# XingqunQi-lab/EmotionGestures

Hardware: AMD Instinct MI355X
Metric: gesture clips/sec (34 frames, 43 joints) (higher is better)
Workload: dtype bf16x3; 1 GPU; TED clips: 4 s 16 kHz audio -> mel(128x124) -> CVAE sample -> generator -> 34x126 pose; global_batch=64, variant=Models_spatial_memory, parallelism=clip-sharded x1, no data-path collective, launch=hipGraph replay, 4 step(s) in flight, branch_streams=False, fold_affine=False

## Files before the change

### emotiongestures_amd/csrc/conv.hip

```cpp
#include <type_traits>
#include "common.h"


namespace {

struct ConvArgs {
    const float* x; const float* w; const float* bias; const float* scale; const float* shift;
    float* y; float* gap;
    float* gap2 = nullptr;
    int H, W, Ho, Wo, cout, relu, nchw, tiles_x, tiles;
    const float* gate = nullptr; const float* res = nullptr; int relu2 = 0;
    const float* in_scale = nullptr; const float* in_shift = nullptr;
    int wrow = 0;
    const unsigned* res_bits = nullptr;
    const float* res_q = nullptr;
    unsigned int* dbg = nullptr;
    const float* sc_x = nullptr; const bf8* sc_whi = nullptr; const bf8* sc_wlo = nullptr; const float* sc_vec = nullptr;
    int sc_H = 0, sc_W = 0, sc_S = 2, sc_B = 0;
};
__device__ __forceinline__ f4 residual_quad(const float* __restrict__ res, const unsigned* __restrict__ bits, size_t e) {
    f4 r = *reinterpret_cast<const f4*>(res + e);
    if (bits) {
        const unsigned nb = bits[e >> 5] >> (unsigned)(e & 28);
        r[0] = (nb & 1u) ? r[0] : 0.f;
        r[1] = (nb & 2u) ? r[1] : 0.f;
        r[2] = (nb & 4u) ? r[2] : 0.f;
        r[3] = (nb & 8u) ? r[3] : 0.f;
    }
    return r;
}

template <int S, int TH> struct ConvGeom {
    static constexpr int IH = (TH - 1) * S + 3;
    static constexpr int IW = 31 * S + 3;
    static constexpr int NPIX = IH * IW;
    static constexpr int PL = (S == 1) ? ((NPIX + 15) / 16 * 16) : (NPIX | 1);
    static constexpr int MT = TH * 2 / 4;
};

template <int TH> struct ConvGeomDG2 {
    static constexpr int IH = TH + 1;
    static constexpr int IW = 33;
    static constexpr int NPIX = IH * IW;
    static constexpr int PL = (NPIX + 15) / 16 * 16;
};

template <int CIN, int NT, int S, int TH>
__global__ __launch_bounds__(256) void conv3x3_f32_kernel(ConvArgs a) {
    using G = ConvGeom<S, TH>;
    constexpr int COUTP = NT * 16, IW = G::IW, NPIX = G::NPIX, PL = G::PL, MT = G::MT;
    __shared__ f4 tile[8 * PL];

    const int tid = threadIdx.x, wave = tid >> 6, lane = tid & 63, li = lane & 15, kq = lane >> 4;
    int tile_id = blockIdx.x, b = blockIdx.y;
    {
        const int total = gridDim.x * gridDim.y;
        if ((total & 7) == 0) {
            const int lin = blockIdx.y * gridDim.x + blockIdx.x;
            const int log = (lin & 7) * (total >> 3) + (lin >> 3);
            b = log / (int)gridDim.x;
            tile_id = log - b * (int)gridDim.x;
        }
    }
    const int ty = tile_id / a.tiles_x, tx = tile_id - ty * a.tiles_x;
    const int oy0 = ty * TH, ox0 = tx * 32;
    const int iy0 = oy0 * S - 1, ix0 = ox0 * S - 1;

    int pbase[MT];
#pragma unroll
    for (int t = 0; t < MT; ++t) {
        const int id = wave * MT + t;
        pbase[t] = ((id >> 1) * S) * IW + ((id & 1) * 16 + li) * S;
    }
    f4 acc[MT][NT];
#pragma unroll
    for (int t = 0; t < MT; ++t)
#pragma unroll
        for (int n = 0; n < NT; ++n) acc[t][n] = (f4){0.f, 0.f, 0.f, 0.f};

    const f4* __restrict__ w4 = reinterpret_cast<const f4*>(a.w);
    const float* __restrict__ xb = a.x + (size_t)b * a.H * a.W * CIN;

    for (int chunk = 0; chunk < CIN / 32; ++chunk) {
        if (chunk) __syncthreads();
        for (int idx = tid; idx < ((NPIX + 7) / 8) * 64; idx += 256) {
            const int p = (idx >> 6) * 8 + (idx & 7), cq = (idx >> 3) & 7;
            if (p < NPIX) {
                const int iy = p / IW, ix = p - iy * IW;
                const int gy = iy0 + iy, gx = ix0 + ix;
                f4 v = (f4){0.f, 0.f, 0.f, 0.f};
                if (gy >= 0 && gy < a.H && gx >= 0 && gx < a.W)
                    v = *reinterpret_cast<const f4*>(xb + ((size_t)gy * a.W + gx) * CIN + chunk * 32 + cq * 4);
                tile[cq * PL + p] = v;
            }
        }
        __syncthreads();
        const f4* wp = w4 + (size_t)(chunk * 8 + kq) * COUTP + li;
#pragma unroll 1
        for (int kh = 0; kh < 3; ++kh) {
// ... 127 lines not shown
#pragma unroll
        for (int t = 0; t < MT; ++t)
#pragma unroll
            for (int n = 0; n < NT; ++n) acc[ph][t][n] = (f4){0.f, 0.f, 0.f, 0.f};
    const float* xb = a.x + (size_t)b * a.H * a.W * CIN;

    const int wave_u = __builtin_amdgcn_readfirstlane(wave);
    constexpr int PIECES = WIMG / 64;
    constexpr int GTOT = NIMG * PIECES;
    constexpr bool COUNTED = (GTOT % 4 == 0);
    constexpr int GW = GTOT / 4;
    auto issue_rows = [&](const bf8* __restrict__ ihi, const bf8* __restrict__ ilo, int row0, int buf) {
        if constexpr (SPLIT) {
            static_assert(COUNTED, "split instantiations deal whole pieces to the four waves");
            const size_t rbase = (size_t)row0 * a.wrow + c0;
#pragma unroll
            for (int p = 0; p < GW; ++p) {
                const int flat = p * 4 + wave_u;
                const int img = flat / PIECES, piece = flat - img * PIECES;
                const int slot = piece * 64 + lane, oct = slot / COUTP, co = slot - oct * COUTP;
                const bf8* src = (img ? ilo : ihi) + rbase + (size_t)oct * a.wrow + co;
                __builtin_amdgcn_global_load_lds((const __attribute__((address_space(1))) void*)src,
                                                 (__attribute__((address_space(3))) void*)(wring + buf * WBUF + img * WIMG + piece * 64), 16, 0, 0);
            }
            return;
        }
        const size_t gbase = (size_t)row0 * COUTP;
        if constexpr (PIECES % 4 == 0) {
#pragma unroll
            for (int img = 0; img < NIMG; ++img) {
                const bf8* src = (img ? ilo : ihi) + gbase;
#pragma unroll
                for (int p = 0; p < PIECES / 4; ++p) {
                    const int piece = p * 4 + wave_u;
                    __builtin_amdgcn_global_load_lds((const __attribute__((address_space(1))) void*)(src + piece * 64 + lane),
                                                     (__attribute__((address_space(3))) void*)(wring + buf * WBUF + img * WIMG + piece * 64),
                                                     16, 0, 0);
                }
            }
        } else {
#pragma unroll
            for (int p = 0; p < (GTOT + 3) / 4; ++p) {
                const int flat = p * 4 + wave_u;
                if (COUNTED || flat < GTOT) {
                    const int img = flat / PIECES, piece = flat - img * PIECES;
                    const bf8* src = (img ? ilo : ihi) + gbase;
                    __builtin_amdgcn_global_load_lds((const __attribute__((address_space(1))) void*)(src + piece * 64 + lane),
                                                     (__attribute__((address_space(3))) void*)(wring + buf * WBUF + img * WIMG + piece * 64),
                                                     16, 0, 0);
                }
            }
        }
    };
    auto issue_weights = [&](int step, int buf) {
        const int chunk = step / 9, tap = step - chunk * 9;
        issue_rows(whi, wlo, tap * (CIN / 8) + chunk * 4, buf);
    };
    constexpr int NIT = (((NPIX + 7) / 8) * 32 + 255) / 256;
    f4 pv[NIT][2];
    int goff[NIT], lslot[NIT];
    auto set_goff = [&](int toy0, int tox0) {
        const int iy0 = DG2 ? toy0 : toy0 * S - 1, ix0 = DG2 ? tox0 : tox0 * S - 1;
#pragma unroll
        for (int it = 0; it < NIT; ++it) {
            const int idx = tid + it * 256;
            const int p = (idx >> 5) * 8 + (idx & 7), oc = (idx >> 3) & 3;
            const int iy = p / IW, ix = p - iy * IW;
            const int gy = iy0 + iy, gx = ix0 + ix;
            const bool inside = p < NPIX && gy >= 0 && gy < a.H && gx >= 0 && gx < a.W;
            goff[it] = inside ? (gy * a.W + gx) * CIN + oc * 8 : -1;
            lslot[it] = p < NPIX ? oc * PL + p : -1;
        }
    };
    set_goff(oy0, ox0);
    auto load_tile = [&](int chunk) {
#pragma unroll
        for (int it = 0; it < NIT; ++it) {
            pv[it][0] = pv[it][1] = (f4){0.f, 0.f, 0.f, 0.f};
            if (goff[it] >= 0) {
                const float* src = xb + goff[it] + chunk * 32;
                pv[it][0] = *reinterpret_cast<const f4*>(src);
                pv[it][1] = *reinterpret_cast<const f4*>(src + 4);
            }
        }
    };
    const int oc8s = ((tid >> 3) & 3) * 8;
    auto store_tile = [&](int chunk) {
        f4 s0 = (f4){1.f, 1.f, 1.f, 1.f}, s1 = s0, h0 = (f4){0.f, 0.f, 0.f, 0.f}, h1 = h0;
        const bool in_aff = a.in_scale != nullptr;
        if (in_aff) {
            s0 = *reinterpret_cast<const f4*>(a.in_scale + chunk * 32 + oc8s); s1 = *reinterpret_cast<const f4*>(a.in_scale + chunk * 32 + oc8s + 4);
            h0 = *reinterpret_cast<const f4*>(a.in_shift + chunk * 32 + oc8s); h1 = *reinterpret_cast<const f4*>(a.in_shift + chunk * 32 + oc8s + 4);
        }
#pragma unroll
        for (int it = 0; it < NIT; ++it) {
            if (lslot[it] >= 0) {
                if (in_aff && goff[it] >= 0) {
                    pv[it][0] = pv[it][0] * s0 + h0;
                    pv[it][1] = pv[it][1] * s1 + h1;
                }
                bf8 hi, lo;
                split_octet<TERMS == 3>(pv[it][0], pv[it][1], hi, lo);
                tile[lslot[it]] = hi;
                if (TERMS == 3) tile[4 * PL + lslot[it]] = lo;
            }
        }
    };

// ... 64 lines not shown
            for (int it = 0; it < SNIT; ++it) {
                sv[it][0] = sv[it][1] = (f4){0.f, 0.f, 0.f, 0.f};
                if (sgoff[it] >= 0) {
                    const float* src = sxb + sgoff[it] + c * 32;
                    sv[it][0] = *reinterpret_cast<const f4*>(src);
                    sv[it][1] = *reinterpret_cast<const f4*>(src + 4);
                }
            }
        };
        load_sc(0);
        load_tile(0);
#pragma unroll
        for (int c = 0; c < SCC; ++c) {
#pragma unroll
            for (int it = 0; it < SNIT; ++it) {
                bf8 hi, lo;
                split_octet<TERMS == 3>(sv[it][0], sv[it][1], hi, lo);
                tile[sslot[it]] = hi;
                if (TERMS == 3) tile[4 * PL + sslot[it]] = lo;
            }
            if (c + 1 < SCC) load_sc(c + 1);
            __syncthreads();
            read_w(fr[0], 2 - c);
            read_x(fr[0], 4);
            mfma_half(fr[0], 0, 4);
            mfma_half(fr[0], 1, 4);
            __syncthreads();
        }
        if (SCC == 2) issue_weights(1, 1);
        const float* __restrict__ fv = a.sc_vec + (size_t)b * a.cout;
#pragma unroll
        for (int n = 0; n < NT; ++n) {
            const f4 fq = *reinterpret_cast<const f4*>(fv + c0 + (wn * NT + n) * 16 + kq * 4);
#pragma unroll
            for (int t = 0; t < MT; ++t) acc[0][t][n] = acc[0][t][n] * fq;
        }
    } else {
        issue_weights(0, 0);
        if (NSTEP > 1) issue_weights(1, 1);
        load_tile(0);
    }
#pragma unroll 1
    for (int chunk = 0; chunk < CIN / 32; ++chunk) {
        store_tile(chunk);
        if (COUNTED && chunk > 0) {
            wait_vmcnt_imm<GW>();
            wait_lgkmcnt0();
            wg_barrier();
        } else {
            __syncthreads();
        }
        if (chunk + 1 < CIN / 32) load_tile(chunk + 1);
        read_w(fr[0], 0);
        read_x(fr[0], 0);
#pragma unroll
        for (int tap = 0; tap < 9; ++tap) {
            const int step = chunk * 9 + tap;
            const bool more = step + 2 < NSTEP;
            if (more) issue_weights(step + 2, (tap + 2) % 3);
            mfma_half(fr[tap & 1], 0, tap);
            mid_sync(more);
            if (tap < 8) { read_w(fr[(tap + 1) & 1], (tap + 1) % 3); read_x(fr[(tap + 1) & 1], tap + 1); }
            mfma_half(fr[tap & 1], 1, tap);
        }
    }

    if constexpr (DG2) {
        const size_t ohw = (size_t)a.Ho * a.Wo;
        float* __restrict__ yb = a.y + (size_t)b * ohw * a.cout;
        const float* __restrict__ rq = a.res_q ? a.res_q + (size_t)b * a.H * a.W * a.cout : nullptr;
#pragma unroll
        for (int ph = 0; ph < 4; ++ph) {
            const int py = ph >> 1, px = ph & 1;
#pragma unroll
            for (int t = 0; t < MT; ++t) {
                const int id = wm * MT + t;
                const int by = oy0 + (id >> 1), bx = ox0 + (id & 1) * 16 + li;
                const int oy = 2 * by + py, ox = 2 * bx + px;
                if (by < a.H && bx < a.W && oy < a.Ho && ox < a.Wo) {
#pragma unroll
                    for (int n = 0; n < NT; ++n) {
                        const int co = (wn * NT + n) * 16 + kq * 4;
                        if (co < a.cout) {
                            f4 v = acc[ph][t][n];
                            if (ph == 0 && rq) v += *reinterpret_cast<const f4*>(rq + ((size_t)by * a.W + bx) * a.cout + co);
                            *reinterpret_cast<f4*>(yb + ((size_t)oy * a.Wo + ox) * a.cout + co) = v;
                        }
                    }
                }
            }
        }
        return;
    }

    f4 gsum[NT], gsq[NT];
    int pixo[MT];
#pragma unroll
    for (int t = 0; t < MT; ++t) {
        const int id = wm * MT + t;
        const int oy = oy0 + (id >> 1), ox = ox0 + (id & 1) * 16 + li;
        pixo[t] = (oy < a.Ho && ox < a.Wo) ? oy * a.Wo + ox : -1;
    }
    const int hw = a.Ho * a.Wo;
    float* __restrict__ yb = a.y + (size_t)b * hw * a.cout;
#pragma unroll
    for (int n = 0; n < NT; ++n) {
        gsum[n] = (f4){0.f, 0.f, 0.f, 0.f};
        gsq[n] = gsum[n];
        const int co = c0 + (wn * NT + n) * 16 + kq * 4;
        const f4 bi = a.bias ? *reinterpret_cast<const f4*>(a.bias + co) : (f4){0.f, 0.f, 0.f, 0.f};
        f4 sc = a.scale ? *reinterpret_cast<const f4*>(a.scale + co) : (f4){1.f, 1.f, 1.f, 1.f};
        f4 sh = a.shift ? *reinterpret_cast<const f4*>(a.shift + co) : (f4){0.f, 0.f, 0.f, 0.f};
        if constexpr (SCC > 0) {
            const float* __restrict__ qv = a.sc_vec + ((size_t)a.sc_B + b) * a.cout + co;
            sc = *reinterpret_cast<const f4*>(qv);
// ... 7 lines not shown
            f4 v = acc[0][t][n] + bi;
            if (a.relu) {
#pragma unroll
                for (int r = 0; r < 4; ++r) v[r] = fmaxf(v[r], 0.f);
            }
            v = v * sc + sh;
            if (a.gate) v = v * gt;
            if (rb && pixo[t] >= 0 && co < a.cout) v += residual_quad(a.res, a.res_bits, rbase + (size_t)pixo[t] * a.cout + co);
            if (a.relu2) {
#pragma unroll
                for (int r = 0; r < 4; ++r) v[r] = fmaxf(v[r], 0.f);
            }
            if (pixo[t] >= 0) {
                if (!a.nchw) {
                    if (co < a.cout) *reinterpret_cast<f4*>(yb + pixo[t] * a.cout + co) = v;
                } else {
#pragma unroll
                    for (int r = 0; r < 4; ++r)
                        if (co + r < a.cout) yb[(co + r) * hw + pixo[t]] = v[r];
                }
                gsum[n] += v;
                if (a.gap2) gsq[n] += v * v;
            }
        }
    }
    if (a.gap) {
        float* sred = reinterpret_cast<float*>(lds);
#pragma unroll
        for (int n = 0; n < NT; ++n) {
#pragma unroll
            for (int r = 0; r < 4; ++r) {
                float s = gsum[n][r];
                s = row16_sum(s);
                if (li == 0) sred[wm * COUTP + (wn * NT + n) * 16 + kq * 4 + r] = s;
                if (a.gap2) {
                    float q = gsq[n][r];
                    q = row16_sum(q);
                    if (li == 0) sred[(WM + wm) * COUTP + (wn * NT + n) * 16 + kq * 4 + r] = q;
                }
            }
        }
        wait_lgkmcnt0();
        wg_barrier();
        if (tid < (SPLIT ? COUTP : a.cout)) {
            float s = 0.f;
#pragma unroll
            for (int m = 0; m < WM; ++m) s += sred[m * COUTP + tid];
            a.gap[((size_t)b * a.tiles + tile_id) * a.cout + c0 + tid] = s;
            if (a.gap2) {
                float q = 0.f;
#pragma unroll
                for (int m = 0; m < WM; ++m) q += sred[(WM + m) * COUTP + tid];
                a.gap2[((size_t)b * a.tiles + tile_id) * a.cout + c0 + tid] = q;
            }
        }
    }
}

template <int TERMS, int TH = 4, bool STAMP = false>
__global__ __launch_bounds__(256, 2) void conv3x3_c32_persistent_kernel(ConvArgs a, const bf8* __restrict__ whi, const bf8* __restrict__ wlo,
                                                                     int total_tiles, int tiles_per_wg) {
    using G = ConvGeom<1, TH>;
    constexpr int CIN = 32, IW = G::IW, NPIX = G::NPIX, PL = G::PL, MT = TH / 2, NT = 2;
    constexpr int NIMG = (TERMS == 3) ? 2 : 1;
    constexpr int TILE = NIMG * 4 * PL, WTAP = 4 * 32, WIMG = 9 * WTAP;
    static_assert(PL - NPIX >= 8 || TH == 4, "the gap scratch of the 8-row variant lives in the planes' padding slots");
    extern __shared__ __attribute__((aligned(16))) bf8 lds[];
    bf8* tile = lds;
    bf8* wl = lds + TILE;
    float* sred_base = reinterpret_cast<float*>(lds + TILE + NIMG * WIMG);
    const int sred_pitch = (TH == 4) ? 32 : PL * 4;
    float* sred = (TH == 4) ? sred_base : reinterpret_cast<float*>(tile + NPIX);

    const int tid = threadIdx.x, wave = tid >> 6, lane = tid & 63, li = lane & 15, kq = lane >> 4;
    const int wave_u = __builtin_amdgcn_readfirstlane(wave);
    int wg = blockIdx.x;
    if ((gridDim.x & 7) == 0) wg = (blockIdx.x & 7) * (gridDim.x >> 3) + (blockIdx.x >> 3);
    const int NWG = gridDim.x;
    const int t_begin = wg, t_end = total_tiles;
    (void)tiles_per_wg;
    if (t_begin >= t_end) return;

#pragma unroll
    for (int img = 0; img < NIMG; ++img) {
        const bf8* src = img ? wlo : whi;
#pragma unroll
        for (int p = 0; p < 5; ++p) {
            const int piece = p * 4 + wave_u;
            if (piece < WIMG / 64)
                __builtin_amdgcn_global_load_lds((const __attribute__((address_space(1))) void*)(src + piece * 64 + lane),
                                                 (__attribute__((address_space(3))) void*)(wl + img * WIMG + piece * 64), 16, 0, 0);
        }
    }

    constexpr int NIT = (((NPIX + 7) / 8) * 32 + 255) / 256;
    int piy[NIT], pix[NIT], lslot[NIT];
#pragma unroll
    for (int it = 0; it < NIT; ++it) {
        const int idx = tid + it * 256;
        const int p = (idx >> 5) * 8 + (idx & 7), oc = (idx >> 3) & 3;
        piy[it] = p / IW;
        pix[it] = p - piy[it] * IW;
        lslot[it] = p < NPIX ? oc * PL + p : -1;
    }
    const int oc8 = ((tid >> 3) & 3) * 8;
    f4 isc[2] = {(f4){1.f, 1.f, 1.f, 1.f}, (f4){1.f, 1.f, 1.f, 1.f}}, ish[2] = {(f4){0.f, 0.f, 0.f, 0.f}, (f4){0.f, 0.f, 0.f, 0.f}};
// ... 445 lines not shown
template <int CIN, int NTS, int TH, int WM, int WN, int TERMS, int SCC = 0>
int launch_conv_split_t(ConvArgs a, int batch, const bf8* whi, const bf8* wlo, hipStream_t st) {
    constexpr int RING = 3;
    using G = ConvGeom<1, TH>;
    constexpr int NIMG = (TERMS == 3) ? 2 : 1;
    constexpr size_t LDS_BYTES = sizeof(bf8) * (size_t)(NIMG * 4 * G::PL + RING * NIMG * 4 * NTS * 16);
    auto kern = conv3x3_bf16_kernel<CIN, NTS, 1, TH, WM, WN, TERMS, RING, true, false, SCC>;
    if (int rc = eg_ensure_dynamic_lds(reinterpret_cast<const void*>(kern), LDS_BYTES, "conv3x3 (channel split)")) return rc;
    a.wrow = a.cout;
    hipLaunchKernelGGL(kern, dim3(a.tiles, batch, a.cout / (NTS * 16)), dim3(256), LDS_BYTES, st, a, whi, wlo);
    return eg_check_launch("conv3x3 (channel split)");
}
template <int KCH, int NTN, int TH, int WM, int WN>
int launch_dgrad_s2_t(const ConvArgs& a, int batch, const bf8* whi, const bf8* wlo, hipStream_t st) {
    constexpr int RING = 3;
    using G = ConvGeomDG2<TH>;
    constexpr size_t LDS_BYTES = sizeof(bf8) * (size_t)(2 * 4 * G::PL + RING * 2 * 4 * NTN * 16);
    auto kern = conv3x3_bf16_kernel<KCH, NTN, 1, TH, WM, WN, 3, RING, false, true>;
    if (int rc = eg_ensure_dynamic_lds(reinterpret_cast<const void*>(kern), LDS_BYTES, "conv3x3 (stride-2 input gradient)")) return rc;
    dim3 grid(eg_cdiv(a.W, 32) * eg_cdiv(a.H, TH), batch);
    hipLaunchKernelGGL(kern, grid, dim3(256), LDS_BYTES, st, a, whi, wlo);
    return eg_check_launch("conv3x3 (stride-2 input gradient)");
}
int conv_channel_split(int wgs, int max_split) {
    const char* e = getenv("EG_CONV_SPLIT");
    const int forced = (e && e[0]) ? atoi(e) : -1;
    if (forced >= 0) return (forced == 2 || forced == 4) && forced <= max_split ? forced : 1;
    int split = 1;
    while (split < max_split && wgs * split * 2 <= 512) split *= 2;
    return split;
}

int body_channel_split(int batch, int tiles, int cin, int cout, int stride, int precision, int nchw_out) {
    if (!((cin == 64 || cin == 128) && cout == cin && stride == 1 && precision == EG_PREC_BF16X3 && !nchw_out)) return 1;
    return conv_channel_split(tiles * batch, cin == 128 ? 4 : 2);
}

template <int CIN, int NT, int S, int TH, int WM, int WN, int SCC = 0>
int launch_conv(const ConvArgs& a, int batch, int precision, hipStream_t st) {
    dim3 grid(a.tiles, batch), block(256);
    if (precision == EG_PREC_F32) {
        if constexpr (SCC > 0) {
            eg_set_error("conv3x3: the fused downsample shortcut exists in the split-bf16 modes only");
            return EG_ERR_UNSUPPORTED;
        }
        hipLaunchKernelGGL((conv3x3_f32_kernel<CIN, NT, S, TH>), grid, block, 0, st, a);
        return eg_check_launch("conv3x3");
    }
    const size_t f32_floats = (size_t)9 * CIN * NT * 16;
    const bf8* whi = reinterpret_cast<const bf8*>(a.w + f32_floats);
    const bf8* wlo = whi + (size_t)9 * (CIN / 8) * NT * 16;
    if (precision == EG_PREC_BF16X3) return launch_conv_bf16<CIN, NT, S, TH, WM, WN, 3, SCC>(a, whi, wlo, grid, st);
    return launch_conv_bf16<CIN, NT, S, TH, WM, WN, 1, SCC>(a, whi, wlo, grid, st);
}

bool conv32_persistent_enabled() {
    static const bool on = [] { const char* e = getenv("EG_CONV32_PERSISTENT"); return !(e && e[0] == '0'); }();
    return on;
}

template <int TERMS, int TH>
int launch_conv32_persistent_t(const ConvArgs& a, int batch, const bf8* whi, const bf8* wlo, hipStream_t st) {
    using G = ConvGeom<1, TH>;
    constexpr int NIMG = (TERMS == 3) ? 2 : 1;
    constexpr size_t LDS_BYTES = sizeof(bf8) * (size_t)(NIMG * 4 * G::PL + NIMG * 9 * 128) + (TH == 4 ? 2 * 4 * 32 * sizeof(float) : 0);
    auto kern = conv3x3_c32_persistent_kernel<TERMS, TH>;
    if (int rc = eg_ensure_dynamic_lds(reinterpret_cast<const void*>(kern), LDS_BYTES, "conv3x3 (32 -> 32, persistent)")) return rc;
    const int total = a.tiles * batch;
    const int cap = 512;
    int grid = total < cap ? total : cap;
    int tpw = eg_cdiv(total, grid);
    grid = eg_cdiv(total, tpw);
    if (grid >= 8) grid = (int)eg_round_up(grid, 8);
    hipLaunchKernelGGL(kern, dim3(grid), dim3(256), LDS_BYTES, st, a, whi, wlo, total, tpw);
    return eg_check_launch("conv3x3 (32 -> 32, persistent)");
}
int launch_conv32_persistent(const ConvArgs& a, int batch, int precision, int th, hipStream_t st) {
    const size_t f32_floats = (size_t)9 * 32 * 32;
    const bf8* whi = reinterpret_cast<const bf8*>(a.w + f32_floats);
    const bf8* wlo = whi + (size_t)9 * 4 * 32;
    static const bool stamp = [] { const char* e = getenv("EG_CONV32_STAMP"); return e && e[0] == '1'; }();
    if (stamp && precision == EG_PREC_BF16X3 && th == 4) {
        static unsigned int* dbg = nullptr;
        const int nwords = 512 * 4 * 8;
        if (!dbg && hipMalloc(&dbg, nwords * sizeof(unsigned int)) != hipSuccess) return EG_ERR_HIP;
        (void)hipMemsetAsync(dbg, 0, nwords * sizeof(unsigned int), st);
        ConvArgs b = a;
        b.dbg = dbg;
        constexpr size_t LDS_BYTES = sizeof(bf8) * (size_t)(2 * 4 * ConvGeom<1, 4>::PL + 2 * 9 * 128) + 2 * 4 * 32 * sizeof(float);
        auto kern = conv3x3_c32_persistent_kernel<3, 4, true>;
        if (int rc = eg_ensure_dynamic_lds(reinterpret_cast<const void*>(kern), LDS_BYTES, "conv3x3 (stamps)")) return rc;
        const int total = a.tiles * batch;
        int grid = total < 512 ? total : 512;
        grid = eg_cdiv(total, eg_cdiv(total, grid));
        if (grid >= 8) grid = (int)eg_round_up(grid, 8);
        hipLaunchKernelGGL(kern, dim3(grid), dim3(256), LDS_BYTES, st, b, whi, wlo, total, 0);
        static unsigned int host[512 * 4 * 8];
        if (hipMemcpyAsync(host, dbg, sizeof(host), hipMemcpyDeviceToHost, st) != hipSuccess || hipStreamSynchronize(st) != hipSuccess) return EG_ERR_HIP;
        double sum[6] = {0, 0, 0, 0, 0, 0};
        int nw = 0;
        for (int w = 0; w < grid * 4; ++w) {
            if (host[w * 8 + 3] == 0) continue;
            ++nw;
            for (int i = 0; i < 6; ++i) sum[i] += host[w * 8 + i];
        }
        const double tiles_per_wave = (double)total / grid;
// ... 82 lines not shown
                     int32_t relu, int32_t nchw_out, int32_t precision, void* stream, const float* in_scale, const float* in_shift, const uint32_t* res_bits,
                     const ShortcutArgs* sc) {
    EG_REQUIRE(x && w && y && batch > 0 && h > 0 && wdt > 0, EG_ERR_BAD_ARG, "eg_conv3x3: null pointer or empty shape");
    EG_REQUIRE(!res_bits || (residual && !gate && ((size_t)batch * h * wdt * cout) % 32 == 0), EG_ERR_BAD_ARG,
               "eg_conv3x3_res_masked: the bit mask needs a residual, no gate and a map of a multiple of 32 elements");
    EG_REQUIRE((in_scale == nullptr) == (in_shift == nullptr) && (!in_scale || (precision != EG_PREC_F32 && cin % 32 == 0 && eg_aligned16(in_scale) &&
               eg_aligned16(in_shift))), EG_ERR_BAD_ARG, "eg_conv3x3: the input affine needs both vectors, a split-bf16 mode and cin %% 32 == 0");
    EG_REQUIRE(!gate || residual, EG_ERR_BAD_ARG, "eg_conv3x3_se: a gate needs a residual");
    EG_REQUIRE(!residual || (!nchw_out && stride == 1 && cout % 4 == 0 && (!gate || eg_aligned16(gate)) && eg_aligned16(residual) && residual != y),
               EG_ERR_BAD_ARG, "eg_conv3x3_se: the fused residual needs NHWC output, stride 1, cout %% 4 == 0 and a residual buffer distinct from y");
    EG_REQUIRE(eg_aligned16(x) && eg_aligned16(w) && eg_aligned16(y), EG_ERR_ALIGN, "eg_conv3x3: pointers must be 16-byte aligned");
    EG_REQUIRE(stride == 1 || stride == 2, EG_ERR_UNSUPPORTED, "eg_conv3x3: stride %d", stride);
    EG_REQUIRE(precision >= 0 && precision <= 2, EG_ERR_BAD_ARG, "eg_conv3x3: precision %d", precision);
    EG_REQUIRE(nchw_out || (cout % 4 == 0), EG_ERR_UNSUPPORTED, "eg_conv3x3: NHWC output needs cout %% 4 == 0");
    ConvArgs a;
    a.x = x; a.w = w; a.bias = bias; a.scale = scale; a.shift = shift; a.y = y; a.gap = gap_partial; a.gap2 = gap_sq;
    a.gate = gate; a.res = residual; a.relu2 = gate ? 1 : 0;
    a.res_bits = res_bits;
    a.in_scale = in_scale; a.in_shift = in_shift;
    a.H = h; a.W = wdt; a.Ho = (h + 2 - 3) / stride + 1; a.Wo = (wdt + 2 - 3) / stride + 1;
    a.cout = cout; a.relu = relu; a.nchw = nchw_out;
    const int th = conv_tile_rows(cin, cout, stride);
    a.tiles_x = eg_cdiv(a.Wo, 32);
    a.tiles = a.tiles_x * eg_cdiv(a.Ho, th);
    hipStream_t st = (hipStream_t)stream;
    const int coutp = (int)eg_round_up(cout, 16);
    EgProfScope prof((int64_t)cin * 1000000 + (int64_t)cout * 1000 + stride * 100 + 1,
                     2.0 * 9 * cin * cout * (double)a.Ho * a.Wo * batch, st);
    if (sc) {
        EG_REQUIRE(precision != EG_PREC_F32 && stride == 1 && !nchw_out && cout == cin && (cin == 64 || cin == 128) && sc->cin * 2 == cin, EG_ERR_UNSUPPORTED,
                   "conv3x3: the fused downsample shortcut serves 32 -> 64 and 64 -> 128 block entries in the split-bf16 modes (cin=%d cout=%d shortcut cin=%d)",
                   cin, cout, sc->cin);
        EG_REQUIRE(sc->x && sc->wimg && sc->vec && !gate && !residual && !bias && !relu && !gap_sq && !in_scale && sc->stride >= 1 &&
                   (sc->h - 1) / sc->stride + 1 == h && (sc->w - 1) / sc->stride + 1 == wdt && eg_aligned16(sc->x) && eg_aligned16(sc->wimg) &&
                   eg_aligned16(sc->vec), EG_ERR_BAD_ARG, "conv3x3: fused downsample shortcut: null / misaligned operand or a block input that does not map onto the output");
        a.sc_x = sc->x; a.sc_vec = sc->vec; a.sc_H = sc->h; a.sc_W = sc->w; a.sc_S = sc->stride; a.sc_B = batch;
        a.sc_whi = reinterpret_cast<const bf8*>(sc->wimg);
        a.sc_wlo = a.sc_whi + (size_t)(sc->cin / 8) * cout;
        a.scale = a.shift = nullptr;
        a.relu2 = 1;
        const int split = body_channel_split(batch, a.tiles, cin, cout, 1, precision, 0);
        const bf8* whi = reinterpret_cast<const bf8*>(a.w + (size_t)9 * cin * cout);
        const bf8* wlo = whi + (size_t)9 * (cin / 8) * cout;
        if (cin == 64 && split == 2) return launch_conv_split_t<64, 2, 8, 4, 1, 3, 1>(a, batch, whi, wlo, st);
        if (cin == 64) return launch_conv<64, 4, 1, 8, 4, 1, 1>(a, batch, precision, st);
        if (split == 2) return launch_conv_split_t<128, 4, 4, 2, 2, 3, 2>(a, batch, whi, wlo, st);
        if (split == 4) return launch_conv_split_t<128, 2, 4, 2, 2, 3, 2>(a, batch, whi, wlo, st);
        return launch_conv<128, 8, 1, 4, 2, 2, 2>(a, batch, precision, st);
    }
    if (cin == 32 && coutp == 32 && cout == 32 && stride == 1 && precision != EG_PREC_F32 && !nchw_out && conv32_persistent_enabled())
        return launch_conv32_persistent(a, batch, precision, th, st);
    if (cin == 32 && coutp == 32 && stride == 1 && th == 4) return launch_conv<32, 2, 1, 4, 4, 1>(a, batch, precision, st);
    if (cin == 32 && coutp == 32 && stride == 1) return launch_conv<32, 2, 1, 8, 4, 1>(a, batch, precision, st);
    if (cin == 32 && coutp == 64 && stride == 2) return launch_conv<32, 4, 2, 2, 2, 2>(a, batch, precision, st);
    if (const int split = body_channel_split(batch, a.tiles, cin, cout, stride, precision, nchw_out); split > 1) {
        const size_t f32_floats = (size_t)9 * cin * cout;
        const bf8* whi = reinterpret_cast<const bf8*>(a.w + f32_floats);
        const bf8* wlo = whi + (size_t)9 * (cin / 8) * cout;
        if (cin == 64 && split == 2) return launch_conv_split_t<64, 2, 8, 4, 1, 3>(a, batch, whi, wlo, st);
        if (cin == 128 && split == 2) return launch_conv_split_t<128, 4, 4, 2, 2, 3>(a, batch, whi, wlo, st);
        if (cin == 128 && split == 4) return launch_conv_split_t<128, 2, 4, 2, 2, 3>(a, batch, whi, wlo, st);
    }
    if (cin == 64 && coutp == 64 && stride == 1) return launch_conv<64, 4, 1, 8, 4, 1>(a, batch, precision, st);
    if (cin == 64 && coutp == 128 && stride == 2) return launch_conv<64, 8, 2, 2, 2, 2>(a, batch, precision, st);
    if (cin == 64 && coutp == 128 && stride == 1) return launch_conv<64, 8, 1, 4, 2, 2>(a, batch, precision, st);
    if (cin == 128 && coutp == 128 && stride == 1) return launch_conv<128, 8, 1, 4, 2, 2>(a, batch, precision, st);
    if (cin == 128 && coutp == 256 && stride == 2) return launch_conv<128, 16, 2, 2, 1, 4>(a, batch, precision, st);
    if (cin == 256 && coutp == 256 && stride == 1) return launch_conv<256, 16, 1, 2, 1, 4>(a, batch, precision, st);
    if (cin == 128 && coutp <= 64 && stride == 1) {
        if (coutp <= 48) return launch_conv<128, 3, 1, 4, 4, 1>(a, batch, precision, st);
        return launch_conv<128, 4, 1, 4, 4, 1>(a, batch, precision, st);
    }
    if (cin == 128 && coutp <= 128 && stride == 1) return launch_conv<128, 8, 1, 4, 2, 2>(a, batch, precision, st);
    eg_set_error("eg_conv3x3: unsupported channels cin=%d cout=%d stride=%d", cin, cout, stride);
    return EG_ERR_UNSUPPORTED;
}
}

extern "C" int eg_conv3x3_dgrad_s2(const float* dy, const float* w_flip, const float* res_q, float* dx, int32_t batch, int32_t h, int32_t wdt, int32_t cin,
                                   int32_t cout, int32_t precision, void* stream) {
    EG_REQUIRE(dy && w_flip && dx && batch > 0 && h > 0 && wdt > 0, EG_ERR_BAD_ARG, "eg_conv3x3_dgrad_s2: null pointer or empty shape");
    EG_REQUIRE(precision == EG_PREC_BF16X3, EG_ERR_UNSUPPORTED, "eg_conv3x3_dgrad_s2: split-bf16 arithmetic only (precision %d)", precision);
    EG_REQUIRE(eg_aligned16(dy) && eg_aligned16(w_flip) && eg_aligned16(dx) && (!res_q || eg_aligned16(res_q)), EG_ERR_ALIGN,
               "eg_conv3x3_dgrad_s2: pointers must be 16-byte aligned");
    ConvArgs a;
    a.x = dy; a.w = w_flip; a.bias = nullptr; a.scale = nullptr; a.shift = nullptr; a.y = dx; a.gap = nullptr;
    a.H = (h - 1) / 2 + 1; a.W = (wdt - 1) / 2 + 1; a.Ho = h; a.Wo = wdt;
    a.cout = cin; a.relu = 0; a.nchw = 0; a.tiles_x = eg_cdiv(a.W, 32); a.tiles = 0;
    a.res_q = res_q;
    hipStream_t st = (hipStream_t)stream;
    const size_t f32_floats = (size_t)9 * cout * cin;
    const bf8* whi = reinterpret_cast<const bf8*>(w_flip + f32_floats);
    const bf8* wlo = whi + (size_t)9 * (cout / 8) * cin;
    EgProfScope prof((int64_t)cin * 1000000 + (int64_t)cout * 1000 + 200 + 8, 2.0 * 9 * cin * cout * (double)a.H * a.W * batch, st);
    if (cin == 32 && cout == 64) return launch_dgrad_s2_t<64, 2, 4, 4, 1>(a, batch, whi, wlo, st);
    if (cin == 64 && cout == 128) return launch_dgrad_s2_t<128, 4, 2, 2, 2>(a, batch, whi, wlo, st);
    if (cin == 128 && cout == 256) return launch_dgrad_s2_t<256, 8, 1, 1, 4>(a, batch, whi, wlo, st);
    eg_set_error("eg_conv3x3_dgrad_s2: unsupported channels %d -> %d", cin, cout);
    return EG_ERR_UNSUPPORTED;
}

extern "C" int eg_stem_conv(const float* x, const float* w9xc, const float* bias, const float* scale, const float* shift,
                            float* y, int32_t batch, int32_t h, int32_t wdt, int32_t c, void* stream) {
    EG_REQUIRE(x && w9xc && bias && scale && shift && y && batch > 0, EG_ERR_BAD_ARG, "eg_stem_conv: null pointer");
    EG_REQUIRE(c % 4 == 0 && c <= 128 && 256 % (c / 4) == 0, EG_ERR_UNSUPPORTED, "eg_stem_conv: C=%d", c);
    hipLaunchKernelGGL(stem_conv_kernel, dim3(batch * h), dim3(256), 3 * (wdt + 2) * sizeof(float), (hipStream_t)stream, x, w9xc, bias, scale, shift, y,
                       batch, h, wdt, c);
    return eg_check_launch("stem_conv");
}

extern "C" int eg_se_gate(const float* gap_partial, int32_t tiles, const float* w1, const float* b1, const float* w2,
                          const float* b2, float* gate, int32_t batch, int32_t c, int32_t hw, void* stream) {
    EG_REQUIRE(gap_partial && w1 && b1 && w2 && b2 && gate && batch > 0, EG_ERR_BAD_ARG, "eg_se_gate: null pointer");
    EG_REQUIRE(c % 8 == 0 && c <= 256 && (c <= 128 ? 128 % c : 256 % c) == 0, EG_ERR_UNSUPPORTED, "eg_se_gate: C=%d", c);
    hipLaunchKernelGGL(se_gate_kernel, dim3(batch), dim3(c <= 128 ? 128 : 256), 0, (hipStream_t)stream, gap_partial, tiles, w1, b1, w2, b2,
                       gate, c, 1.0f / (float)hw);
// ... 76 lines not shown
```

Measured before the change: 27230 clips/s.

## Add phase-plane stride-2 conv3x3 kernel that streams input planes per tap group

Adds a new stride-2 3x3 conv kernel that splits the input tile into four parity planes and loads one plane at a time. Taps are reordered so each plane is consumed before the next is stored, which overlaps the plane loads with MFMA work and shrinks the LDS tile compared with the interleaved stride-2 layout. The existing kernel also gets the same tap reordering. The new path is chosen for cin 32/64 stride-2 layers when the grid is large enough, with an env override. The cost is a more complex vmcnt/barrier schedule that is easy to get wrong.

New measurement: 27540 clips/s (median of 6 runs). 1.1% higher.

```diff
diff --git a/emotiongestures_amd/csrc/conv.hip b/emotiongestures_amd/csrc/conv.hip
--- a/emotiongestures_amd/csrc/conv.hip
+++ b/emotiongestures_amd/csrc/conv.hip
@@ -1,3 +1,4 @@
+#include <string.h>
 #include <type_traits>
 #include "common.h"
 
@@ -45,6 +46,9 @@
     static constexpr int PL = (NPIX + 15) / 16 * 16;
 };
 
+constexpr int s2p_tap(int k) { constexpr int T[9] = {4, 3, 5, 1, 7, 0, 2, 6, 8}; return T[k]; }
+constexpr int s2p_plane(int k) { constexpr int P[9] = {0, 1, 1, 2, 2, 3, 3, 3, 3}; return P[k]; }
+
 template <int CIN, int NT, int S, int TH>
 __global__ __launch_bounds__(256) void conv3x3_f32_kernel(ConvArgs a) {
     using G = ConvGeom<S, TH>;
@@ -278,8 +282,9 @@
             }
         }
     };
+    auto tap_of = [](int k) { return (S == 2 && !DG2) ? s2p_tap(k) : k; };
     auto issue_weights = [&](int step, int buf) {
-        const int chunk = step / 9, tap = step - chunk * 9;
+        const int chunk = step / 9, tap = tap_of(step - chunk * 9);
         issue_rows(whi, wlo, tap * (CIN / 8) + chunk * 4, buf);
     };
     constexpr int NIT = (((NPIX + 7) / 8) * 32 + 255) / 256;
@@ -450,7 +455,7 @@
         }
         if (chunk + 1 < CIN / 32) load_tile(chunk + 1);
         read_w(fr[0], 0);
-        read_x(fr[0], 0);
+        read_x(fr[0], tap_of(0));
 #pragma unroll
         for (int tap = 0; tap < 9; ++tap) {
             const int step = chunk * 9 + tap;
@@ -458,7 +463,7 @@
             if (more) issue_weights(step + 2, (tap + 2) % 3);
             mfma_half(fr[tap & 1], 0, tap);
             mid_sync(more);
-            if (tap < 8) { read_w(fr[(tap + 1) & 1], (tap + 1) % 3); read_x(fr[(tap + 1) & 1], tap + 1); }
+            if (tap < 8) { read_w(fr[(tap + 1) & 1], (tap + 1) % 3); read_x(fr[(tap + 1) & 1], tap_of(tap + 1)); }
             mfma_half(fr[tap & 1], 1, tap);
         }
     }
@@ -572,6 +577,250 @@
 #pragma unroll
                 for (int m = 0; m < WM; ++m) q += sred[(WM + m) * COUTP + tid];
                 a.gap2[((size_t)b * a.tiles + tile_id) * a.cout + c0 + tid] = q;
+            }
+        }
+    }
+}
+
+template <int TH> struct ConvGeomS2P {
+    static constexpr int PW = 33;
+    static constexpr int NPIX = (TH + 1) * PW;
+    static constexpr int PL = (NPIX + 15) / 16 * 16;
+};
+
+template <int CIN, int NTT, int TH, int WM, int WN, int TERMS, bool AFF>
+__global__ __launch_bounds__(256, 2) void conv3x3_s2_planes_kernel(ConvArgs a, const bf8* __restrict__ whi, const bf8* __restrict__ wlo) {
+    using G = ConvGeomS2P<TH>;
+    constexpr int COUTP = NTT * 16, PW = G::PW, NPIX = G::NPIX, PL = G::PL;
+    constexpr int MT = TH * 2 / WM, NT = NTT / WN;
+    constexpr int NIMG = (TERMS == 3) ? 2 : 1;
+    constexpr int TILE = NIMG * 4 * PL;
+    constexpr int WIMG = 4 * COUTP;
+    constexpr int WBUF = NIMG * WIMG;
+    constexpr int NSTEP = (CIN / 32) * 9;
+    static_assert(WM * WN == 4 && MT == 4 && NT * WN == NTT, "a wave owns one 2 x 32 output block (four pixel tiles) of its channel range");
+    extern __shared__ __attribute__((aligned(16))) bf8 lds[];
+    bf8* tile = lds;
+    bf8* wring = lds + TILE;
+
+    const int tid = threadIdx.x, wave = tid >> 6, lane = tid & 63, li = lane & 15, kq = lane >> 4;
+    const int wm = wave / WN, wn = wave % WN;
+    int tile_id = blockIdx.x, b = blockIdx.y;
+    {
+        const int total = gridDim.x * gridDim.y;
+        if ((total & 7) == 0) {
+            const int lin = blockIdx.y * gridDim.x + blockIdx.x;
+            const int log = (lin & 7) * (total >> 3) + (lin >> 3);
+            b = log / (int)gridDim.x;
+            tile_id = log - b * (int)gridDim.x;
+        }
+    }
+    const int ty = tile_id / a.tiles_x, tx = tile_id - ty * a.tiles_x;
+    const int oy0 = ty * TH, ox0 = tx * 32;
+
+    int pbase[MT];
+#pragma unroll
+    for (int t = 0; t < MT; ++t) pbase[t] = (2 * wm + (t >> 1)) * PW + (t & 1) * 16 + li;
+    f4 acc[MT][NT];
+#pragma unroll
+    for (int t = 0; t < MT; ++t)
+#pragma unroll
+        for (int n = 0; n < NT; ++n) acc[t][n] = (f4){0.f, 0.f, 0.f, 0.f};
+    const float* xb = a.x + (size_t)b * a.H * a.W * CIN;
+
+    const int wave_u = __builtin_amdgcn_readfirstlane(wave);
+    constexpr int PIECES = WIMG / 64;
+    static_assert(PIECES % 4 == 0, "every wave copies PIECES / 4 pieces of each image (the per-step wait is a counted vmcnt)");
+    constexpr int GW = NIMG * PIECES / 4;
+    const unsigned lane_b = lane * (unsigned)sizeof(bf8);
+    auto issue_weights = [&](int step, int buf) {
+        const int chunk = step / 9, tap = s2p_tap(step - chunk * 9);
+        const size_t gbase = (size_t)(tap * (CIN / 8) + chunk * 4) * COUTP;
+#pragma unroll
+        for (int img = 0; img < NIMG; ++img) {
+            const bf8* src = (img ? wlo : whi) + gbase;
+#pragma unroll
+            for (int p = 0; p < PIECES / 4; ++p) {
+                const int piece = p * 4 + wave_u;
+                __builtin_amdgcn_global_load_lds((const __attribute__((address_space(1))) void*)(reinterpret_cast<const char*>(src + piece * 64) + lane_b),
+                                                 (__attribute__((address_space(3))) void*)(wring + buf * WBUF + img * WIMG + piece * 64), 16, 0, 0);
+            }
+        }
+    };
+    constexpr int NIT = (((NPIX + 7) / 8) * 32 + 255) / 256;
+    constexpr int LV = 2 * NIT;
+    static_assert(PL > NPIX, "the spare slot");
+    f4 pv[NIT][2];
+    int goff[NIT], pmask = 0;
+    static_assert(NIT * 4 <= 32, "one mask word");
+#pragma unroll
+    for (int it = 0; it < NIT; ++it) {
+        const int idx = tid + it * 256;
+        const int p = (idx >> 5) * 8 + (idx & 7), oc = (idx >> 3) & 3;
+        const int pr = p / PW, pc = p - pr * PW;
+        const int gy0 = 2 * (oy0 + pr), gx0 = 2 * (ox0 + pc);
+        goff[it] = (gy0 * a.W + gx0) * CIN + oc * 8;
+#pragma unroll
+        for (int pl = 0; pl < 4; ++pl) {
+            const int rp = pl >> 1, cp = pl & 1, gy = gy0 - rp, gx = gx0 - cp;
+            if (p < NPIX && pr < TH + rp && pc < 32 + cp && gy >= 0 && gy < a.H && gx >= 0 && gx < a.W) pmask |= 1 << (it * 4 + pl);
+        }
+    }
+    auto load_plane = [&](int chunk, int pl) {
+        const int poff = ((pl >> 1) * a.W + (pl & 1)) * CIN - chunk * 32;
+#pragma unroll
+        for (int it = 0; it < NIT; ++it) {
+            const float* src = xb + (((pmask >> (it * 4 + pl)) & 1) ? goff[it] - poff : 0);
+            pv[it][0] = *reinterpret_cast<const f4*>(src);
+            pv[it][1] = *reinterpret_cast<const f4*>(src + 4);
+        }
+    };
+    const int ocs = (tid >> 3) & 3, oc8s = ocs * 8, p0 = (tid >> 5) * 8 + (tid & 7);
+    auto store_plane = [&](int chunk, int pl) {
+        f4 s0, s1, h0, h1;
+        if constexpr (AFF) {
+            s0 = *reinterpret_cast<const f4*>(a.in_scale + chunk * 32 + oc8s); s1 = *reinterpret_cast<const f4*>(a.in_scale + chunk * 32 + oc8s + 4);
+            h0 = *reinterpret_cast<const f4*>(a.in_shift + chunk * 32 + oc8s); h1 = *reinterpret_cast<const f4*>(a.in_shift + chunk * 32 + oc8s + 4);
+        }
+#pragma unroll
+        for (int it = 0; it < NIT; ++it) {
+            const u32x4_t m = (u32x4_t)(0u - (unsigned)((pmask >> (it * 4 + pl)) & 1));
+            f4 x0 = pv[it][0], x1 = pv[it][1];
+            if constexpr (AFF) { x0 = x0 * s0 + h0; x1 = x1 * s1 + h1; }
+            const f4 v0 = __builtin_bit_cast(f4, __builtin_bit_cast(u32x4_t, x0) & m), v1 = __builtin_bit_cast(f4, __builtin_bit_cast(u32x4_t, x1) & m);
+            bf8 hi, lo;
+            split_octet<TERMS == 3>(v0, v1, hi, lo);
+            const int p = p0 + it * 64, slot = ocs * PL + (p < PL - 1 ? p : PL - 1);
+            tile[slot] = hi;
+            if (TERMS == 3) tile[4 * PL + slot] = lo;
+        }
+    };
+
+    struct Frags { bf8 wh[NT], wl[NT], xh[MT], xl[MT]; };
+    auto read_w = [&](Frags& f, int slot) {
+        const bf8* Wh = wring + slot * WBUF + kq * COUTP + wn * NT * 16 + li;
+#pragma unroll
+        for (int n = 0; n < NT; ++n) {
+            f.wh[n] = Wh[n * 16];
+            if (TERMS == 3) f.wl[n] = Wh[WIMG + n * 16];
+        }
+    };
+    auto read_x = [&](Frags& f, int tap) {
+        const int toff = (tap / 3 == 2 ? PW : 0) + (tap % 3 == 2 ? 1 : 0);
+#pragma unroll
+        for (int t = 0; t < MT; ++t) {
+            f.xh[t] = tile[kq * PL + pbase[t] + toff];
+            if (TERMS == 3) f.xl[t] = tile[(4 + kq) * PL + pbase[t] + toff];
+        }
+    };
+    auto mfma_half = [&](const Frags& f, int half) {
+#pragma unroll
+        for (int t = half * (MT / 2); t < (half + 1) * (MT / 2); ++t)
+#pragma unroll
+            for (int n = 0; n < NT; ++n) {
+                if (TERMS == 3) {
+                    acc[t][n] = __builtin_amdgcn_mfma_f32_16x16x32_bf16(f.wl[n], f.xh[t], acc[t][n], 0, 0, 0);
+                    acc[t][n] = __builtin_amdgcn_mfma_f32_16x16x32_bf16(f.wh[n], f.xl[t], acc[t][n], 0, 0, 0);
+                }
+                acc[t][n] = __builtin_amdgcn_mfma_f32_16x16x32_bf16(f.wh[n], f.xh[t], acc[t][n], 0, 0, 0);
+            }
+    };
+    auto mid_sync = [&](int k, bool nxt) {
+        __builtin_amdgcn_sched_barrier(0);
+        if (k <= 4) wait_vmcnt_imm<GW + LV>();
+        else if (k <= 6) { if (nxt) wait_vmcnt_imm<GW + LV>(); else wait_vmcnt_imm<GW>(); }
+        else { if (nxt) wait_vmcnt_imm<GW>(); else wait_vmcnt_imm<0>(); }
+        wait_lgkmcnt0();
+        wg_barrier();
+    };
+    Frags fr[2];
+    issue_weights(0, 0);
+    issue_weights(1, 1);
+    load_plane(0, 0);
+    store_plane(0, 0);
+    wait_vmcnt_imm<0>();
+    wait_lgkmcnt0();
+    wg_barrier();
+    issue_weights(2, 2);
+    __builtin_amdgcn_sched_barrier(0);
+    load_plane(0, 1);
+    read_w(fr[0], 0);
+    read_x(fr[0], s2p_tap(0));
+#pragma unroll 1
+    for (int chunk = 0; chunk < CIN / 32; ++chunk) {
+        int chunk_u = chunk;
+        asm volatile("" : "+s"(chunk_u), "+v"(pmask));
+        const bool nxt = chunk_u + 1 < CIN / 32;
+#pragma unroll
+        for (int k = 0; k < 9; ++k) {
+            const int step = chunk_u * 9 + k;
+            const bool after_swap = k == 0 || k == 1 || k == 3 || k == 5;
+            const bool swap = k == 0 || k == 2 || k == 4 || (k == 8 && nxt);
+            const int kn = (k + 1) % 9, fn = k < 8 ? (k + 1) & 1 : 0;
+            if (!after_swap && step + 2 < NSTEP) issue_weights(step + 2, (k + 2) % 3);
+            mfma_half(fr[k & 1], 0);
+            mid_sync(k, nxt);
+            if (swap) {
+                store_plane(k < 8 ? chunk_u : chunk_u + 1, s2p_plane(kn));
+                mfma_half(fr[k & 1], 1);
+                wait_lgkmcnt0();
+                wg_barrier();
+                issue_weights(step + 3, k % 3);
+                __builtin_amdgcn_sched_barrier(0);
+                if (k == 0) load_plane(chunk_u, 2);
+                else if (k == 2) load_plane(chunk_u, 3);
+                else if (k == 8) load_plane(chunk_u + 1, 1);
+                else if (nxt) load_plane(chunk_u + 1, 0);
+                read_w(fr[fn], kn % 3);
+                read_x(fr[fn], s2p_tap(kn));
+            } else {
+                if (k < 8) { read_w(fr[fn], kn % 3); read_x(fr[fn], s2p_tap(kn)); }
+                mfma_half(fr[k & 1], 1);
+            }
+        }
+    }
+
+    int pixo[MT];
+#pragma unroll
+    for (int t = 0; t < MT; ++t) {
+        const int oy = oy0 + 2 * wm + (t >> 1), ox = ox0 + (t & 1) * 16 + li;
+        pixo[t] = (oy < a.Ho && ox < a.Wo) ? oy * a.Wo + ox : -1;
+    }
+    const int hw = a.Ho * a.Wo;
+    float* __restrict__ yb = a.y + (size_t)b * hw * COUTP;
+    const bool blk_ok = oy0 + 2 * wm < a.Ho;
+    const size_t gbase = ((size_t)b * a.tiles + (size_t)(ty * (TH / 2) + wm) * a.tiles_x + tx) * COUTP;
+#pragma unroll
+    for (int n = 0; n < NT; ++n) {
+        f4 gsum[2], gsq[2];
+        gsum[0] = gsum[1] = gsq[0] = gsq[1] = (f4){0.f, 0.f, 0.f, 0.f};
+        const int co = (wn * NT + n) * 16 + kq * 4;
+        const f4 bi = a.bias ? *reinterpret_cast<const f4*>(a.bias + co) : (f4){0.f, 0.f, 0.f, 0.f};
+        const f4 sc = a.scale ? *reinterpret_cast<const f4*>(a.scale + co) : (f4){1.f, 1.f, 1.f, 1.f};
+        const f4 sh = a.shift ? *reinterpret_cast<const f4*>(a.shift + co) : (f4){0.f, 0.f, 0.f, 0.f};
+#pragma unroll
+        for (int t = 0; t < MT; ++t) {
+            f4 v = acc[t][n] + bi;
+            if (a.relu) {
+#pragma unroll
+                for (int r = 0; r < 4; ++r) v[r] = fmaxf(v[r], 0.f);
+            }
+            v = v * sc + sh;
+            if (pixo[t] >= 0) {
+                *reinterpret_cast<f4*>(yb + pixo[t] * COUTP + co) = v;
+                gsum[t >> 1] += v;
+                if (a.gap2) gsq[t >> 1] += v * v;
+            }
+        }
+        if (a.gap) {
+#pragma unroll
+            for (int r = 0; r < 4; ++r) {
+                gsum[0][r] = (0.f + row16_sum(gsum[0][r])) + row16_sum(gsum[1][r]);
+                if (a.gap2) gsq[0][r] = (0.f + row16_sum(gsq[0][r])) + row16_sum(gsq[1][r]);
+            }
+            if (li == 0 && blk_ok) {
+                *reinterpret_cast<f4*>(a.gap + gbase + co) = gsum[0];
+                if (a.gap2) *reinterpret_cast<f4*>(a.gap2 + gbase + co) = gsq[0];
             }
         }
     }
@@ -1123,6 +1372,37 @@
     const bf8* wlo = whi + (size_t)9 * (CIN / 8) * NT * 16;
     if (precision == EG_PREC_BF16X3) return launch_conv_bf16<CIN, NT, S, TH, WM, WN, 3, SCC>(a, whi, wlo, grid, st);
     return launch_conv_bf16<CIN, NT, S, TH, WM, WN, 1, SCC>(a, whi, wlo, grid, st);
+}
+
+template <int CIN, int NTT, int TH, int WM, int WN>
+int launch_conv_s2_planes(const ConvArgs& a, int batch, int precision, hipStream_t st) {
+    using G = ConvGeomS2P<TH>;
+    const bf8* whi = reinterpret_cast<const bf8*>(a.w + (size_t)9 * CIN * NTT * 16);
+    const bf8* wlo = whi + (size_t)9 * (CIN / 8) * NTT * 16;
+    const dim3 grid(a.tiles_x * eg_cdiv(a.Ho, TH), batch);
+    auto go = [&](auto kern, size_t lds_bytes) {
+        if (int rc = eg_ensure_dynamic_lds(reinterpret_cast<const void*>(kern), lds_bytes, "conv3x3 (stride 2, planes)")) return rc;
+        hipLaunchKernelGGL(kern, grid, dim3(256), lds_bytes, st, a, whi, wlo);
+        return eg_check_launch("conv3x3 (stride 2, planes)");
+    };
+    constexpr size_t LDS3 = sizeof(bf8) * (size_t)(2 * 4 * G::PL + 3 * 2 * 4 * NTT * 16), LDS1 = sizeof(bf8) * (size_t)(4 * G::PL + 3 * 4 * NTT * 16);
+    if (a.in_scale) {
+        if (precision == EG_PREC_BF16X3) return go(conv3x3_s2_planes_kernel<CIN, NTT, TH, WM, WN, 3, true>, LDS3);
+        return go(conv3x3_s2_planes_kernel<CIN, NTT, TH, WM, WN, 1, true>, LDS1);
+    }
+    if (precision == EG_PREC_BF16X3) return go(conv3x3_s2_planes_kernel<CIN, NTT, TH, WM, WN, 3, false>, LDS3);
+    return go(conv3x3_s2_planes_kernel<CIN, NTT, TH, WM, WN, 1, false>, LDS1);
+}
+int conv_s2_form(int cin, int batch, int ho, int wo) {
+    const char* e = getenv("EG_CONV_S2");
+    if (e && !strcmp(e, "interleaved")) return 0;
+    const bool forced = e && !strncmp(e, "planes", 6);
+    const int wgs = eg_cdiv(wo, 32) * eg_cdiv(ho, cin == 64 ? 4 : 8) * batch;
+    if (!forced && wgs < 256) return 0;
+    if (cin == 64) return 4;
+    if (e && !strcmp(e, "planes4")) return 4;
+    if (e && !strcmp(e, "planes8")) return 8;
+    return wgs >= 512 ? 8 : 4;
 }
 
 bool conv32_persistent_enabled() {
@@ -1311,6 +1591,10 @@
         return launch_conv32_persistent(a, batch, precision, th, st);
     if (cin == 32 && coutp == 32 && stride == 1 && th == 4) return launch_conv<32, 2, 1, 4, 4, 1>(a, batch, precision, st);
     if (cin == 32 && coutp == 32 && stride == 1) return launch_conv<32, 2, 1, 8, 4, 1>(a, batch, precision, st);
+    const int s2p = (stride == 2 && cout == coutp && precision != EG_PREC_F32 && !nchw_out && (!gap_partial || eg_aligned16(gap_partial)) &&
+                     (!gap_sq || eg_aligned16(gap_sq))) ? conv_s2_form(cin, batch, a.Ho, a.Wo) : 0;
+    if (cin == 32 && coutp == 64 && stride == 2 && s2p == 8) return launch_conv_s2_planes<32, 4, 8, 4, 1>(a, batch, precision, st);
+    if (cin == 32 && coutp == 64 && stride == 2 && s2p == 4) return launch_conv_s2_planes<32, 4, 4, 2, 2>(a, batch, precision, st);
     if (cin == 32 && coutp == 64 && stride == 2) return launch_conv<32, 4, 2, 2, 2, 2>(a, batch, precision, st);
     if (const int split = body_channel_split(batch, a.tiles, cin, cout, stride, precision, nchw_out); split > 1) {
         const size_t f32_floats = (size_t)9 * cin * cout;
@@ -1321,6 +1605,7 @@
         if (cin == 128 && split == 4) return launch_conv_split_t<128, 2, 4, 2, 2, 3>(a, batch, whi, wlo, st);
     }
     if (cin == 64 && coutp == 64 && stride == 1) return launch_conv<64, 4, 1, 8, 4, 1>(a, batch, precision, st);
+    if (cin == 64 && coutp == 128 && stride == 2 && s2p == 4) return launch_conv_s2_planes<64, 8, 4, 2, 2>(a, batch, precision, st);
     if (cin == 64 && coutp == 128 && stride == 2) return launch_conv<64, 8, 2, 2, 2, 2>(a, batch, precision, st);
     if (cin == 64 && coutp == 128 && stride == 1) return launch_conv<64, 8, 1, 4, 2, 2>(a, batch, precision, st);
     if (cin == 128 && coutp == 128 && stride == 1) return launch_conv<128, 8, 1, 4, 2, 2>(a, batch, precision, st);
```
